# xu-ji/IIC

Hardware: AMD Instinct MI355X
Metric: paired-images/sec, STL10 96x96 ClusterNet5g+IID_loss (higher is better)
Workload: dtype bf16; 1 GPU; STL10 96x96 ClusterNet5g IID+ (cluster_sobel.py train step), batch 660 pairs/GPU, 5 sub-heads, k=70, bf16 MFMA convs / fp32 stem+heads+loss, fused HIP Adam; global_batch_pairs=660, input=96x96x1 grey -> sobel 2ch, parallelism=dp1, streams=2, launch=hip-graph replay: 6 linear graph segments, the two views on two streams

## Files before the change

iic_amd/csrc/conv_igemm_p64.hip:

```cpp
#include "common.h"
#include "conv_plan.h"
#include "conv_tile.h"
#include "../../include/iic_hip.h"

#define P64_BM 256
#define P64_BN 64
#define P64_THREADS 512
#define P64_NT 9
#define P64_CLD P64_BN
#define P64_SC_BYTES(BM_) ((BM_) * P64_CLD * 2)
#define P64_NTAB 4
#define P64_TAB_BYTES(BM_) (P64_NTAB * (BM_) * (4 + 2))

struct P64Walk {
  int n, y, x;
};
__device__ __forceinline__ void p64_walk_init(P64Walk& w, const iic_conv_geom& g, int m) {
  const int plane = g.MY * g.MX;
  w.n = m / plane;
  const int r = m - w.n * plane;
  w.y = r / g.MX;
  w.x = r - w.y * g.MX;
}
__device__ __forceinline__ void p64_walk_advance(P64Walk& w, const iic_conv_geom& g, int d_y, int d_x) {
  w.x += d_x;
  w.y += d_y;
  if (w.x >= g.MX) { w.x -= g.MX; ++w.y; }
  while (w.y >= g.MY) { w.y -= g.MY; ++w.n; }
}
__device__ __forceinline__ void p64_walk_pixels(const P64Walk& w, const iic_conv_geom& g, int& pin,
                                                int& pout) {
  const bool valid = w.n < g.N;
  const int n = valid ? w.n : g.N - 1, y = valid ? w.y : g.MY - 1, x = valid ? w.x : g.MX - 1;
  pin = (n * g.in_Hp + y * g.sy + g.oy) * g.in_Wp + x * g.sx + g.ox;
  pout = valid ? (n * g.out_Hp + y * g.ty + g.py) * g.out_Wp + x * g.tx + g.px : -1;
}

struct P64Row {
  int n, y, x, pin, pout;
};
struct P64Step {
  int d_n, d_y, d_x, MY, MX, pin_step, pin_xw, pin_yw, pout_step, pout_xw, pout_yw;
};
__device__ __forceinline__ void p64_row_init(P64Row& r, const iic_conv_geom& g, int m) {
  P64Walk w;
  p64_walk_init(w, g, m);
  r.n = w.n; r.y = w.y; r.x = w.x;
  r.pin = (w.n * g.in_Hp + w.y * g.sy + g.oy) * g.in_Wp + w.x * g.sx + g.ox;
  r.pout = (w.n * g.out_Hp + w.y * g.ty + g.py) * g.out_Wp + w.x * g.tx + g.px;
}
__device__ __forceinline__ void p64_row_advance(P64Row& r, const P64Step& s) {
  r.n += s.d_n; r.y += s.d_y; r.x += s.d_x; r.pin += s.pin_step; r.pout += s.pout_step;
  const bool cx = r.x >= s.MX;
  r.x -= cx ? s.MX : 0; r.y += cx ? 1 : 0; r.pin += cx ? s.pin_xw : 0; r.pout += cx ? s.pout_xw : 0;
  const bool cy = r.y >= s.MY;
  r.y -= cy ? s.MY : 0; r.n += cy ? 1 : 0; r.pin += cy ? s.pin_yw : 0; r.pout += cy ? s.pout_yw : 0;
}

__device__ __forceinline__ void p64_dma16s(unsigned voff, const unsigned char* sbase, unsigned lds_dst) {
  unsigned keep;
  asm volatile(
      "s_mov_b32 %0, m0\n\ts_mov_b32 m0, %3\n\ts_nop 0\n\tglobal_load_lds_dwordx4 %1, %2\n\ts_mov_b32 m0, %0"
      : "=&s"(keep)
      : "v"(voff), "s"(sbase), "s"(lds_dst)
      : "memory");
}

template <int ABL, int RED, bool FORM>
__global__ __launch_bounds__(512) void conv_igemm_p64_kernel(
    const iic_conv_geom g, const bf16_t* __restrict__ in, const unsigned char* __restrict__ wfrag,
    bf16_t* __restrict__ out, float* __restrict__ stats, const bf16_t* __restrict__ res_grad,
    const bf16_t* __restrict__ res_act, int accumulate, int num_tiles, int pb_bytes, int max_tap_off,
    const bf16_t* __restrict__ red_y, const float* __restrict__ red_coef,
    const bf16_t* __restrict__ red_y2, float* __restrict__ red_stats, float* __restrict__ red_stats2,
    unsigned long long* __restrict__ prof) {
  constexpr bool PROF = (ABL & 8) != 0;
  constexpr bool BK = FORM && RED == 0;
  constexpr int NW = 8, BM = P64_BM;
  constexpr int NWM = BM / 64;
  constexpr int SC_BYTES = BM * P64_CLD * 2, TAB_ROWS = P64_NTAB * BM;
  unsigned long long ph[6] = {0, 0, 0, 0, 0, 0}, t_a = 0, t_b = 0, t_loop = 0;
  extern __shared__ __attribute__((aligned(16))) unsigned char smem_raw[];
  unsigned char* const sP0 = smem_raw;
  unsigned char* const sP1 = smem_raw + pb_bytes;
  bf16_t* const sC = reinterpret_cast<bf16_t*>(smem_raw + 2 * pb_bytes);
  int* const s_pout = reinterpret_cast<int*>(smem_raw + 2 * pb_bytes + SC_BYTES);
  unsigned short* const s_prow = reinterpret_cast<unsigned short*>(s_pout + TAB_ROWS);
  float* const s_red = reinterpret_cast<float*>(sC);

  constexpr int NTH = NW * 64;
  constexpr int NCO = 1;
  const int tid = threadIdx.x, lane = tid & 63;
  const int wave = __builtin_amdgcn_readfirstlane(tid >> 6);
  const int wm = wave >> 1, wn = wave & 1;
  const int l31 = lane & 31, g5 = lane >> 5;
  const uint32_t g5x = (uint32_t)g5 << 4;
  typedef const bf16x8 __attribute__((address_space(3))) * lds_frag_ptr;
  const uint32_t lds_base = __builtin_amdgcn_readfirstlane(
      (uint32_t)(uintptr_t)(__attribute__((address_space(3))) unsigned char*)smem_raw);
  const int M = g.N * g.MY * g.MX;
  const int in_pixels = g.N * g.in_Hp * g.in_Wp;

  const int G = gridDim.x;
  const int wl = xcd_tile_index(blockIdx.x, G);
  const int t0 = (int)(((long)wl * num_tiles) / G), t1 = (int)(((long)(wl + 1) * num_tiles) / G);
  if (t0 >= t1) return;

  const int v_tapoff = g.tap_off[lane & (IIC_MAX_TAPS - 1)];
  const int d_y = BM / g.MX, d_x = BM - d_y * g.MX;

  P64Walk wr, w0, w255;
  p64_walk_init(wr, g, t0 * BM + (tid & (BM - 1)));
  p64_walk_init(w0, g, t0 * BM);
  p64_walk_init(w255, g, t0 * BM + BM - 1);
  int plo_q[3], nblk_q[3];
  auto tabulate = [&](int t) {
    int pin, pout, p0, p255, dummy;
    p64_walk_pixels(w0, g, p0, dummy);
    p64_walk_pixels(w255, g, p255, dummy);
    p0 = __builtin_amdgcn_readfirstlane(p0);
    p255 = __builtin_amdgcn_readfirstlane(p255);
    if (tid < BM) {
      p64_walk_pixels(wr, g, pin, pout);
      s_pout[(t & (P64_NTAB - 1)) * BM + tid] = pout;
      s_prow[(t & (P64_NTAB - 1)) * BM + tid] = (unsigned short)(pin - p0);
    }
    p64_walk_advance(wr, g, d_y, d_x);
    p64_walk_advance(w0, g, d_y, d_x);
    p64_walk_advance(w255, g, d_y, d_x);
    plo_q[0] = plo_q[1];
    nblk_q[0] = nblk_q[1];
    plo_q[1] = plo_q[2];
    nblk_q[1] = nblk_q[2];
    plo_q[2] = p0;
    nblk_q[2] = ((p255 + max_tap_off - p0 + 1) * 128 + 1023) >> 10;
  };
  auto dma_issue = [&](unsigned char* dst, int plo, int nblk) {
    for (int blk = wave; blk < nblk; blk += NW) {
      const int q = blk * 64 + lane;
      const int r = q >> 3;
      const int ls = (q & 7) ^ ((r >> 1) & 7);
      int p = plo + r;
      p = p < in_pixels ? p : in_pixels - 1;
      __builtin_amdgcn_global_load_lds(
          (const __attribute__((address_space(1))) void*)(in + ((long)p * 64 + ls * 8)),
          (__attribute__((address_space(3))) void*)(dst + blk * 1024), 16, 0, 0);
    }
  };

  P64Step stp;
  P64Row rr, r0, r255;
  int pin_last = 0;
  uint32_t lane_src = 0;
  if (BK) {
    const int plane = g.MY * g.MX;
    stp.d_n = BM / plane;
    const int rem = BM - stp.d_n * plane;
    stp.d_y = rem / g.MX;
    stp.d_x = rem - stp.d_y * g.MX;
    stp.MY = g.MY; stp.MX = g.MX;
    stp.pin_step = (stp.d_n * g.in_Hp + stp.d_y * g.sy) * g.in_Wp + stp.d_x * g.sx;
    stp.pin_xw = g.sy * g.in_Wp - g.MX * g.sx;
    stp.pin_yw = (g.in_Hp - g.MY * g.sy) * g.in_Wp;
    stp.pout_step = (stp.d_n * g.out_Hp + stp.d_y * g.ty) * g.out_Wp + stp.d_x * g.tx;
    stp.pout_xw = g.ty * g.out_Wp - g.MX * g.tx;
    stp.pout_yw = (g.out_Hp - g.MY * g.ty) * g.out_Wp;
    pin_last = ((g.N - 1) * g.in_Hp + (g.MY - 1) * g.sy + g.oy) * g.in_Wp + (g.MX - 1) * g.sx + g.ox;
    p64_row_init(rr, g, t0 * BM + (tid & (BM - 1)));
    p64_row_init(r0, g, t0 * BM);
    p64_row_init(r255, g, t0 * BM + BM - 1);
    lane_src = (uint32_t)(lane >> 3) * 128u + (uint32_t)(((lane & 7) ^ (lane >> 4) ^ ((wave & 1) << 2)) << 4);
  }
  auto tabulate1 = [&](int t) {
    const int p0 = r0.n < g.N ? r0.pin : pin_last;
    const int p255 = r255.n < g.N ? r255.pin : pin_last;
    if (wave < BM / 64) {
      const bool valid = rr.n < g.N;
      s_pout[(t & (P64_NTAB - 1)) * BM + tid] = valid ? rr.pout : -1;
      s_prow[(t & (P64_NTAB - 1)) * BM + tid] = (unsigned short)((valid ? rr.pin : pin_last) - p0);
      p64_row_advance(rr, stp);
    }
    p64_row_advance(r0, stp);
    p64_row_advance(r255, stp);
    plo_q[0] = plo_q[1];
    nblk_q[0] = nblk_q[1];
    plo_q[1] = plo_q[2];
    nblk_q[1] = nblk_q[2];
    plo_q[2] = p0;
    nblk_q[2] = ((p255 + max_tap_off - p0 + 1) * 128 + 1023) >> 10;
  };
  auto dma_issue1 = [&](uint32_t dst, int plo, int nblk) {
    const unsigned char* const ing = reinterpret_cast<const unsigned char*>(in);
    for (int blk = wave; blk < nblk; blk += NW) {
      const int rb = plo + blk * 8;
      const unsigned char* src = ing + (long)rb * 128;
      uint32_t vo = lane_src;
      if (rb + 7 >= in_pixels) {
        const int rc = rb < in_pixels ? rb : in_pixels - 1;
        int p = rb + (lane >> 3);
        p = p < in_pixels ? p : in_pixels - 1;
        src = ing + (long)rc * 128;
        vo = (uint32_t)(p - rc) * 128u + (lane_src & 127u);
      }
      p64_dma16s(vo, src, dst + (uint32_t)blk * 1024u);
    }
  };
  int R0[2];

  if (BK) {
    tabulate1(t0);
    tabulate1(t0 + 1);
    __syncthreads();
#pragma unroll
    for (int ms = 0; ms < 2; ++ms) R0[ms] = s_prow[(t0 & (P64_NTAB - 1)) * BM + wm * 64 + ms * 32 + l31];
    dma_issue1(lds_base, plo_q[1], nblk_q[1]);
  } else {
    tabulate(t0);
    tabulate(t0 + 1);
    dma_issue(sP0, plo_q[1], nblk_q[1]);
  }
  u32x4 Bw[P64_NT][NCO][4];
#pragma unroll
  for (int tap = 0; tap < P64_NT; ++tap)
#pragma unroll
    for (int c = 0; c < NCO; ++c) {
      const unsigned char* p = wfrag + ((long)g.tap_w[tap] * 2 + wn + c) * 4096 + lane * 16;
#pragma unroll
      for (int ks = 0; ks < 4; ++ks) Bw[tap][c][ks] = *reinterpret_cast<const u32x4*>(p + ks * 1024);
    }
  f32x2 st_s[NCO], st_ss[NCO];
#pragma unroll
  for (int c = 0; c < NCO; ++c) {
    st_s[c] = f32x2{0.f, 0.f};
    st_ss[c] = f32x2{0.f, 0.f};
  }
  TileRed tr;
  if (RED) tile_red_zero(tr);

  if (PROF) t_loop = __builtin_readcyclecounter();
  for (int t = t0; t < t1; ++t) {
    const int par = (t - t0) & 1;
    unsigned char* const sP = par ? sP1 : sP0;
    if (PROF) t_a = __builtin_readcyclecounter();
    asm volatile("s_waitcnt vmcnt(0)" ::: "memory");
    __syncthreads();
    if (PROF) { t_b = __builtin_readcyclecounter(); ph[0] += t_b - t_a; t_a = t_b; }
    const bool spread = RED == 0 && !res_grad && !res_act && !accumulate;
    if (t > t0 && !(ABL & 2) && !spread)
      igemm_store_tile<P64_BN, BM, NTH, 0, RED, (RED ? 1 : 4)>(sC, s_pout + ((t - 1) & (P64_NTAB - 1)) * BM,
                                                            out, res_grad, res_act, accumulate, P64_BN, 0, tid,
                                                            red_y, red_coef, red_y2, &tr);
    if (PROF) { t_b = __builtin_readcyclecounter(); ph[1] += t_b - t_a; t_a = t_b; }
    if (!BK) {
      if (t + 1 < t1 && !(ABL & 1)) dma_issue(par ? sP0 : sP1, plo_q[2], nblk_q[2]);
      tabulate(t + 2);
    }
    if (PROF) { t_b = __builtin_readcyclecounter(); ph[2] += t_b - t_a; t_a = t_b; }
    if (!BK) {
#pragma unroll
      for (int ms = 0; ms < 2; ++ms)
        R0[ms] = s_prow[(t & (P64_NTAB - 1)) * BM + wm * 64 + ms * 32 + l31];
    }
    const uint32_t pbase = lds_base + (par ? (uint32_t)pb_bytes : 0u);
    const int prow = (int)(pbase >> 7);
    const uint32_t kfix = (pbase >> 4) & 0x40u;
    f32x16 acc[2][NCO];
    constexpr int NTAPS = (ABL & 4) ? 1 : P64_NT;
    auto load_a = [&](int tap, bf16x8 (&a)[2][4]) {
      const int toff = __builtin_amdgcn_readlane(v_tapoff, tap);
      if (FORM) {
        const int toffp = toff + prow;
#pragma unroll
        for (int ms = 0; ms < 2; ++ms) {
          uint32_t tt = (uint32_t)(R0[ms] + toffp) << 3;
          asm volatile("" : "+v"(tt));
          uint32_t u = (tt << 4) | (tt & 0x70u);
          asm volatile("" : "+v"(u));
#pragma unroll
          for (int ks = 0; ks < 4; ++ks)
            a[ms][ks] = *reinterpret_cast<const lds_frag_ptr>((uintptr_t)(u ^ g5x ^ ((uint32_t)(ks << 5) ^ kfix)));
        }
        return;
      }
#pragma unroll
      for (int ms = 0; ms < 2; ++ms) {
        const int R = R0[ms] + toff;
        const int key = (R >> 1) & 7;
        const int base = R * 128 + (((g5 ^ key) & 1) << 4);
        const int kk = (key >> 1) << 5;
#pragma unroll
        for (int ks = 0; ks < 4; ++ks)
          a[ms][ks] = *reinterpret_cast<const bf16x8*>(sP + base + ((ks << 5) ^ kk));
      }
    };
#pragma unroll
    for (int tap = 0; tap < NTAPS; ++tap) {
      bf16x8 a[2][4];
      load_a(tap, a);
      if (BK) {
        if (tap == 0 && t + 1 < t1 && !(ABL & 1)) dma_issue1(lds_base + (par ? 0u : (uint32_t)pb_bytes), plo_q[2], nblk_q[2]);
        if (tap == (NTAPS > 6 ? 6 : NTAPS - 1)) tabulate1(t + 2);
      }
      if (spread && t > t0 && !(ABL & 2)) {
        constexpr int SIT = BM * 8 / NTH;
        constexpr int PER = (SIT + P64_NT - 2) / (P64_NT - 1);
#pragma unroll
        for (int q = 0; q < PER; ++q) {
          const int it = (tap - 1) * PER + q;
          if (tap >= 1 && it < SIT) {
            const int idx = tid + it * NTH;
            const int row = idx >> 3, ch = idx & 7;
            const int po = s_pout[((t - 1) & (P64_NTAB - 1)) * BM + row];
            if (po >= 0)
              *reinterpret_cast<uint4*>(out + (long)po * P64_BN + ch * 8) =
                  *reinterpret_cast<const uint4*>(sC + row * P64_CLD + ch * 8);
          }
        }
      }
#pragma unroll
      for (int ks = 0; ks < 4; ++ks)
#pragma unroll
        for (int c = 0; c < NCO; ++c) {
          const bf16x8 b = __builtin_bit_cast(bf16x8, Bw[tap][c][ks]);
          if (tap == 0 && ks == 0) {
            const f32x16 z = {0.f, 0.f, 0.f, 0.f, 0.f, 0.f, 0.f, 0.f, 0.f, 0.f, 0.f, 0.f, 0.f, 0.f, 0.f, 0.f};
            acc[0][c] = __builtin_amdgcn_mfma_f32_32x32x16_bf16(a[0][ks], b, z, 0, 0, 0);
            acc[1][c] = __builtin_amdgcn_mfma_f32_32x32x16_bf16(a[1][ks], b, z, 0, 0, 0);
          } else {
            acc[0][c] = __builtin_amdgcn_mfma_f32_32x32x16_bf16(a[0][ks], b, acc[0][c], 0, 0, 0);
            acc[1][c] = __builtin_amdgcn_mfma_f32_32x32x16_bf16(a[1][ks], b, acc[1][c], 0, 0, 0);
          }
        }
    }
    if (stats) {
      if ((t + 1) * BM > M) {
#pragma unroll
        for (int ms = 0; ms < 2; ++ms)
#pragma unroll
          for (int r = 0; r < 16; ++r)
            if (t * BM + wm * 64 + ms * 32 + mfma32_row(r, lane) >= M) {
#pragma unroll
              for (int c = 0; c < NCO; ++c) acc[ms][c][r] = 0.f;
            }
      }
#pragma unroll
      for (int c = 0; c < NCO; ++c)
#pragma unroll
        for (int ms = 0; ms < 2; ++ms)
#pragma unroll
          for (int r = 0; r < 16; r += 2) {
            const f32x2 v = {acc[ms][c][r], acc[ms][c][r + 1]};
            st_s[c] += v;
            st_ss[c] += v * v;
          }
    }
    if (PROF) { t_b = __builtin_readcyclecounter(); ph[3] += t_b - t_a; t_a = t_b; }
    asm volatile("s_waitcnt lgkmcnt(0)" ::: "memory");
    __builtin_amdgcn_s_barrier();
    if (PROF) { t_b = __builtin_readcyclecounter(); ph[4] += t_b - t_a; t_a = t_b; }
#pragma unroll
    for (int c = 0; c < NCO; ++c)
#pragma unroll
      for (int ms = 0; ms < 2; ++ms)
#pragma unroll
        for (int r = 0; r < 16; ++r)
          sC[(wm * 64 + ms * 32 + mfma32_row(r, lane)) * P64_CLD + (wn + c) * 32 + l31] = f32_to_bf16(acc[ms][c][r]);
    if (BK && t + 1 < t1) {
#pragma unroll
      for (int ms = 0; ms < 2; ++ms) R0[ms] = s_prow[((t + 1) & (P64_NTAB - 1)) * BM + wm * 64 + ms * 32 + l31];
    }
    if (PROF) { t_b = __builtin_readcyclecounter(); ph[5] += t_b - t_a; }
  }
  if (PROF && prof && tid == 0) {
    unsigned long long* q = prof + (long)blockIdx.x * 8;
#pragma unroll
    for (int i = 0; i < 6; ++i) q[i] = ph[i];
    q[6] = (unsigned long long)(t1 - t0);
    q[7] = __builtin_readcyclecounter() - t_loop;
  }

  __syncthreads();
  if (!(ABL & 2))
    igemm_store_tile<P64_BN, BM, NTH, 0, RED, (RED ? 1 : 4)>(sC, s_pout + ((t1 - 1) & (P64_NTAB - 1)) * BM, out,
                                                          res_grad, res_act, accumulate, P64_BN, 0, tid,
                                                          red_y, red_coef, red_y2, &tr);
  if (RED)
    igemm_red_finish<P64_BN, NTH, RED>(tr, reinterpret_cast<float*>(sC), red_stats, red_stats2, P64_BN,
                                               0, tid);
  if (stats) {
    __syncthreads();
#pragma unroll
    for (int c = 0; c < NCO; ++c) {
      float s1 = st_s[c][0] + st_s[c][1], s2 = st_ss[c][0] + st_ss[c][1];
      s1 += __shfl_xor(s1, 32, 64);
      s2 += __shfl_xor(s2, 32, 64);
      if (lane < 32) {
        s_red[(wm * 2 + 0) * P64_BN + (wn + c) * 32 + lane] = s1;
        s_red[(wm * 2 + 1) * P64_BN + (wn + c) * 32 + lane] = s2;
      }
    }
    __syncthreads();
    if (tid < P64_BN) {
      float a0 = 0.f, a1 = 0.f;
#pragma unroll
      for (int q = 0; q < NWM; ++q) {
        a0 += s_red[(q * 2 + 0) * P64_BN + tid];
        a1 += s_red[(q * 2 + 1) * P64_BN + tid];
      }
      const int stripe = blockIdx.x % IIC_STAT_STRIPES;
      iic_stat_add(stats, stripe, P64_BN, tid, 0, a0);
      iic_stat_add(stats, stripe, P64_BN, tid, 1, a1);
    }
  }
}

#ifdef IIC_DEBUG_HOOKS
static unsigned long long* g_p64_prof = nullptr;
IIC_HOOK void iic_debug_p64_prof(void* buf) { g_p64_prof = (unsigned long long*)buf; }
#else
static constexpr unsigned long long* g_p64_prof = nullptr;
#endif
IIC_SWITCH(g_p64_grid, 0, iic_debug_p64_grid)
IIC_SWITCH(g_p64_form, 1, iic_debug_p64_form)

static long p64_pb_bytes(const iic_conv_geom* g, int bm = P64_BM) {
  return (((long)(bm == 128 ? g->NP : g->NP256) * 128) + 1023) & ~1023L;
}

bool iic_p64_plan(const iic_conv_geom* g, conv_plan* p) {
  if (g->Cin != 64 || g->Cout != 64 || g->ntaps != P64_NT || g->NP256 <= 0 || g->NP256 > 65535) return false;
  if (!igemm_dense_host(g)) return false;
  const long lds = 2 * p64_pb_bytes(g) + P64_SC_BYTES(P64_BM) + P64_TAB_BYTES(P64_BM);
  if (lds > IIC_LDS_BYTES) return false;
  const long nt = ((long)g->N * g->MY * g->MX + P64_BM - 1) / P64_BM;
  const int ncu = g_p64_grid > 0 ? g_p64_grid : iic_num_cus();
  p->kernel = CONV_P64;
  p->mtiles = (int)nt;
  p->grid = nt < ncu ? (int)nt : ncu;
  p->lds_a = (int)p64_pb_bytes(g);
  p->lds = lds;
  return true;
}

int iic_p64_launch(const iic_conv_geom* g, const conv_plan& p, const void* in, const void* wfrag, void* out, float* stats,
                   const void* res_grad, const void* res_act, int accumulate, const void* red_y,
                   const float* red_coef, const void* red_y2, float* red_stats, float* red_stats2,
                   void* stream) {
  const int red = red_y ? (red_y2 ? 2 : 1) : 0;
  const long M = (long)g->N * g->MY * g->MX;
  if (M <= 0) return IIC_ERR_ARG;
  if (M >= (1L << 31) - P64_BM || (long)g->N * g->in_Hp * g->in_Wp >= (1L << 31)) return IIC_ERR_UNSUPPORTED;
  int mto = 0;
  for (int i = 0; i < g->ntaps; ++i) mto = g->tap_off[i] > mto ? g->tap_off[i] : mto;
  int rc = IIC_OK;
#define P64_LAUNCH3(AB_, RD_, FM_)                                                                     \
  rc = iic_launch_lds<conv_igemm_p64_kernel<AB_, RD_, FM_>>(                                           \
      dim3(p.grid), dim3(512), p.lds, (hipStream_t)stream, *g, (const bf16_t*)in,                      \
      (const unsigned char*)wfrag, (bf16_t*)out, stats, (const bf16_t*)res_grad,                       \
      (const bf16_t*)res_act, accumulate, p.mtiles, p.lds_a, mto, (const bf16_t*)red_y, red_coef,      \
      (const bf16_t*)red_y2, red_stats, red_stats2, g_p64_prof)
#ifdef IIC_DEBUG_HOOKS
#define P64_LAUNCH2(AB_, RD_)                                                                          \
  do {                                                                                                 \
    if (g_p64_form) P64_LAUNCH3(AB_, RD_, true);                                                       \
    else P64_LAUNCH3(AB_, RD_, false);                                                                 \
  } while (0)
#else
#define P64_LAUNCH2(AB_, RD_) P64_LAUNCH3(AB_, RD_, true)
#endif
#define P64_LAUNCH(AB_) P64_LAUNCH2(AB_, 0)
  if (red == 1) P64_LAUNCH2(0, 1);
  else if (red == 2) P64_LAUNCH2(0, 2);
  else {
    switch (iic_debug_get_ablate()) {
#ifdef IIC_BD_ABLATIONS
      case 1: P64_LAUNCH(1); break;
      case 2: P64_LAUNCH(2); break;
      case 3: P64_LAUNCH(3); break;
      case 4: P64_LAUNCH(4); break;
      case 7: P64_LAUNCH(7); break;
      case 8: P64_LAUNCH(8); break;
#endif
      default: P64_LAUNCH(0); break;
    }
  }
  return rc ? rc : iic_launch_status();
}
```

iic_amd/csrc/conv_tile.h:

```cpp
#pragma once
#include "common.h"
#include "../../include/iic_hip.h"

__device__ __forceinline__ void igemm_row_pixels(const iic_conv_geom& g, int m, int& pin, int& pout) {
  const int plane = g.MY * g.MX;
  const int mp = g.MP > 0 ? g.MP : plane;
  int n = m / mp;
  int r = m - n * mp;
  const bool valid = n < g.N && r < plane;
  if (n >= g.N) { n = g.N - 1; r = plane - 1; }
  r = r < plane ? r : plane - 1;
  const int y = r / g.MX, x = r - y * g.MX;
  pin = (n * g.in_Hp + y * g.sy + g.oy) * g.in_Wp + x * g.sx + g.ox;
  pout = valid ? (n * g.out_Hp + y * g.ty + g.py) * g.out_Wp + x * g.tx + g.px : -1;
}
__device__ __forceinline__ int igemm_rows(const iic_conv_geom& g) {
  return g.N * (g.MP > 0 ? g.MP : g.MY * g.MX);
}
__device__ __forceinline__ bool igemm_tile_has_invalid(const iic_conv_geom& g, int m0, int bm) {
  const int plane = g.MY * g.MX;
  if (m0 + bm > igemm_rows(g)) return true;
  return g.MP > 0 && g.MP != plane && (m0 % g.MP) + bm > plane;
}
static inline long igemm_rows_host(const iic_conv_geom* g) {
  return (long)g->N * (g->MP > 0 ? g->MP : g->MY * g->MX);
}
static inline bool igemm_dense_host(const iic_conv_geom* g) { return g->MP <= 0 || g->MP == g->MY * g->MX; }

#define ROWB 144
#define PT144_ROWS 7
#define PT144_PIECE (PT144_ROWS * ROWB)
static inline long pt144_bytes(long npix) {
  return ((npix + PT144_ROWS - 1) / PT144_ROWS) * PT144_PIECE + 16;
}

__device__ __forceinline__ int xcd_tile_index(int b, int nwg) {
  const int q = nwg >> 3, r = nwg & 7, xcd = b & 7, idx = b >> 3;
  return (xcd < r ? xcd * (q + 1) : r * (q + 1) + (xcd - r) * q) + idx;
}

template <bool GATHER, int NTHREADS, int NB = 4>
__device__ __forceinline__ void igemm_load_patch(unsigned char* sA, const bf16_t* __restrict__ in,
                                                 int Cin, int c0, int p_lo, int npix,
                                                 int in_pixels, const int* s_pin, int tid) {
  const int n8 = npix * 8;
  for (int base = 0; base < n8; base += NTHREADS * NB) {
    u32x4 v[NB];
#pragma unroll
    for (int u = 0; u < NB; ++u) {
      const int idx = base + u * NTHREADS + tid;
      v[u] = (u32x4){0u, 0u, 0u, 0u};
      if (idx < n8) {
        const long p = GATHER ? (long)s_pin[idx >> 3] : (long)p_lo + (idx >> 3);
        if (p < in_pixels) v[u] = *reinterpret_cast<const u32x4*>(in + (p * Cin + c0 + (idx & 7) * 8));
      }
    }
#pragma unroll
    for (int u = 0; u < NB; ++u) {
      const int idx = base + u * NTHREADS + tid;
      if (idx < n8) *reinterpret_cast<u32x4*>(sA + (idx >> 3) * ROWB + (idx & 7) * 16) = v[u];
    }
  }
}

struct TileRed {
  float s[8], sy[8], sy2[8];
};
__device__ __forceinline__ void tile_red_zero(TileRed& r) {
#pragma unroll
  for (int i = 0; i < 8; ++i) r.s[i] = r.sy[i] = r.sy2[i] = 0.f;
}

template <int BN, int BM, int NTHREADS, int PAD = 8, int RED = 0, int UB = 4>
__device__ __forceinline__ void igemm_store_tile(const bf16_t* sC, const int* s_pout,
                                                 bf16_t* __restrict__ out,
                                                 const bf16_t* __restrict__ res_grad,
                                                 const bf16_t* __restrict__ res_act, int accumulate,
                                                 int Cout, int n0, int tid,
                                                 const bf16_t* __restrict__ red_y = nullptr,
                                                 const float* __restrict__ red_coef = nullptr,
                                                 const bf16_t* __restrict__ red_y2 = nullptr,
                                                 TileRed* red = nullptr) {
  constexpr int CLD = BN + PAD;
  constexpr int CH = BN / 8;
  constexpr int ITERS = (BM * CH + NTHREADS - 1) / NTHREADS;
  constexpr int U = ITERS < UB ? ITERS : UB;
  static_assert(NTHREADS % CH == 0, "a thread must keep its channel chunk");
  const bool add_prev = accumulate & IIC_ACC_ADD, premask = accumulate & IIC_ACC_PREMASK;
  const bool any_in = add_prev || res_grad || res_act;
  const int ch = tid % CH;
  float msc[RED ? 8 : 1], msh[RED ? 8 : 1];
  if (RED && red_coef) {
#pragma unroll
    for (int i = 0; i < 8; ++i) {
      msc[RED ? i : 0] = red_coef[n0 + ch * 8 + i];
      msh[RED ? i : 0] = red_coef[Cout + n0 + ch * 8 + i];
    }
  }
  for (int b0 = 0; b0 < ITERS; b0 += U) {
    long o[U];
    uint4 pv[U], gv[U], av[U], yv[U], zv[U];
#pragma unroll
    for (int u = 0; u < U; ++u) {
      const int idx = tid + (b0 + u) * NTHREADS;
      const int row = idx / CH;
      const int po = (idx < BM * CH) ? s_pout[row] : -1;
      o[u] = po < 0 ? -1 : (long)po * Cout + n0 + ch * 8;
      if (o[u] >= 0) {
        if (add_prev) pv[u] = *reinterpret_cast<const uint4*>(out + o[u]);
        if (res_grad) gv[u] = *reinterpret_cast<const uint4*>(res_grad + o[u]);
        if (res_act) av[u] = *reinterpret_cast<const uint4*>(res_act + o[u]);
        if (RED) yv[u] = *reinterpret_cast<const uint4*>(red_y + o[u]);
        if (RED == 2) zv[u] = *reinterpret_cast<const uint4*>(red_y2 + o[u]);
      }
    }
#pragma unroll
    for (int u = 0; u < U; ++u) {
      if (o[u] < 0) continue;
      const int row = (tid + (b0 + u) * NTHREADS) / CH;
      uint4 v = *reinterpret_cast<const uint4*>(sC + row * CLD + ch * 8);
      if (any_in) {
        uint32_t vv[4] = {v.x, v.y, v.z, v.w};
        float f[8];
#pragma unroll
        for (int i = 0; i < 4; ++i) { f[2 * i] = bf16lo(vv[i]); f[2 * i + 1] = bf16hi(vv[i]); }
        if (add_prev) {
          const uint32_t oo[4] = {pv[u].x, pv[u].y, pv[u].z, pv[u].w};
#pragma unroll
          for (int i = 0; i < 4; ++i) { f[2 * i] += bf16lo(oo[i]); f[2 * i + 1] += bf16hi(oo[i]); }
        }
        if (premask) {
          if (res_grad) {
            const uint32_t gg[4] = {gv[u].x, gv[u].y, gv[u].z, gv[u].w};
#pragma unroll
            for (int i = 0; i < 4; ++i) { f[2 * i] += bf16lo(gg[i]); f[2 * i + 1] += bf16hi(gg[i]); }
          }
          if (res_act) {
            const uint32_t aa[4] = {av[u].x, av[u].y, av[u].z, av[u].w};
#pragma unroll
            for (int i = 0; i < 4; ++i) {
              if (!(bf16lo(aa[i]) > 0.f)) f[2 * i] = 0.f;
              if (!(bf16hi(aa[i]) > 0.f)) f[2 * i + 1] = 0.f;
            }
          }
        } else if (res_grad) {
          const uint32_t gg[4] = {gv[u].x, gv[u].y, gv[u].z, gv[u].w};
          const uint32_t aa[4] = {av[u].x, av[u].y, av[u].z, av[u].w};
#pragma unroll
          for (int i = 0; i < 4; ++i) {
            if (bf16lo(aa[i]) > 0.f) f[2 * i] += bf16lo(gg[i]);
            if (bf16hi(aa[i]) > 0.f) f[2 * i + 1] += bf16hi(gg[i]);
          }
        }
        v = make_uint4(pack_bf16x2(f[0], f[1]), pack_bf16x2(f[2], f[3]), pack_bf16x2(f[4], f[5]),
                       pack_bf16x2(f[6], f[7]));
      }
      *reinterpret_cast<uint4*>(out + o[u]) = v;
      if (RED) {
        const uint32_t gq4[4] = {v.x, v.y, v.z, v.w};
        const uint32_t yy[4] = {yv[u].x, yv[u].y, yv[u].z, yv[u].w};
        float gq[8], yq[8];
#pragma unroll
        for (int i = 0; i < 4; ++i) {
          gq[2 * i] = bf16lo(gq4[i]); gq[2 * i + 1] = bf16hi(gq4[i]);
          yq[2 * i] = bf16lo(yy[i]); yq[2 * i + 1] = bf16hi(yy[i]);
        }
        if (red_coef) {
#pragma unroll
          for (int i = 0; i < 8; ++i)
            if (!(yq[i] * msc[RED ? i : 0] + msh[RED ? i : 0] > 0.f)) gq[i] = 0.f;
        }
#pragma unroll
        for (int i = 0; i < 8; ++i) { red->s[i] += gq[i]; red->sy[i] += gq[i] * yq[i]; }
        if (RED == 2) {
          const uint32_t zz[4] = {zv[u].x, zv[u].y, zv[u].z, zv[u].w};
#pragma unroll
          for (int i = 0; i < 4; ++i) {
            red->sy2[2 * i] += gq[2 * i] * bf16lo(zz[i]);
            red->sy2[2 * i + 1] += gq[2 * i + 1] * bf16hi(zz[i]);
          }
        }
      }
    }
  }
}

template <int BN, int NTHREADS, int RED>
__device__ __forceinline__ void igemm_red_finish(TileRed& r, float* scratch, float* red_stats,
                                                 float* red_stats2, int Cout, int n0, int tid) {
  constexpr int CH = BN / 8, NW = NTHREADS / 64;
  static_assert(64 % CH == 0, "channel chunks must divide the wave");
  const int lane = tid & 63, wave = tid >> 6, ch = tid % CH;
#pragma unroll
  for (int i = 0; i < 8; ++i) {
#pragma unroll
    for (int o = CH; o < 64; o <<= 1) {
      r.s[i] += __shfl_xor(r.s[i], o, 64);
      r.sy[i] += __shfl_xor(r.sy[i], o, 64);
      if (RED == 2) r.sy2[i] += __shfl_xor(r.sy2[i], o, 64);
    }
  }
  __syncthreads();
  if (lane < CH) {
#pragma unroll
    for (int i = 0; i < 8; ++i) {
      scratch[(wave * 3 + 0) * BN + ch * 8 + i] = r.s[i];
      scratch[(wave * 3 + 1) * BN + ch * 8 + i] = r.sy[i];
      if (RED == 2) scratch[(wave * 3 + 2) * BN + ch * 8 + i] = r.sy2[i];
    }
  }
  __syncthreads();
  if (tid < BN) {
    float a0 = 0.f, a1 = 0.f, a2 = 0.f;
    for (int w = 0; w < NW; ++w) {
      a0 += scratch[(w * 3 + 0) * BN + tid];
      a1 += scratch[(w * 3 + 1) * BN + tid];
      if (RED == 2) a2 += scratch[(w * 3 + 2) * BN + tid];
    }
    const int stripe = blockIdx.x % IIC_STAT_STRIPES;
    iic_stat_add(red_stats, stripe, Cout, n0 + tid, 0, a0);
    iic_stat_add(red_stats, stripe, Cout, n0 + tid, 1, a1);
    if (RED == 2) {
      iic_stat_add(red_stats2, stripe, Cout, n0 + tid, 0, a0);
      iic_stat_add(red_stats2, stripe, Cout, n0 + tid, 1, a2);
    }
  }
}
```

Before: 19480 paired-images/sec.

## Prefetch epilogue residual/reduction operands during the MFMA phase of the p64 conv

Adds an AHEAD template variant of the p64 implicit-GEMM conv kernel. It issues global loads for the next tile's epilogue inputs (residual grad, activation, accumulate source, reduction y/y2, coefficients) right after the MFMA loop, before the barrier, then consumes them from registers in a new store routine. For RED kernels the accumulators are packed to bf16 early to free registers. The aim is to hide epilogue global-load latency behind the barrier and LDS writes, at the cost of higher VGPR pressure. It is enabled by default for non-spread, RED 0/1 launches.

```diff
diff --git a/iic_amd/csrc/conv_igemm_p64.hip b/iic_amd/csrc/conv_igemm_p64.hip
--- a/iic_amd/csrc/conv_igemm_p64.hip
+++ b/iic_amd/csrc/conv_igemm_p64.hip
@@ -66,7 +66,7 @@
       : "memory");
 }
 
-template <int ABL, int RED, bool FORM>
+template <int ABL, int RED, bool FORM, bool AHEAD>
 __global__ __launch_bounds__(512) void conv_igemm_p64_kernel(
     const iic_conv_geom g, const bf16_t* __restrict__ in, const unsigned char* __restrict__ wfrag,
     bf16_t* __restrict__ out, float* __restrict__ stats, const bf16_t* __restrict__ res_grad,
@@ -236,6 +236,11 @@
   }
   TileRed tr;
   if (RED) tile_red_zero(tr);
+  const bool spread = RED == 0 && !res_grad && !res_act && !accumulate;
+  constexpr int EPI_ITERS = BM * (P64_BN / 8) / NTH;
+  constexpr int EPI_NS = RED == 0 ? EPI_ITERS : (RED == 1 ? 2 : 1);
+  TileEpi<RED, EPI_NS> epi;
+  const bool epi_ahead = AHEAD && !spread && !(ABL & 2);
 
   if (PROF) t_loop = __builtin_readcyclecounter();
   for (int t = t0; t < t1; ++t) {
@@ -245,11 +250,16 @@
     asm volatile("s_waitcnt vmcnt(0)" ::: "memory");
     __syncthreads();
     if (PROF) { t_b = __builtin_readcyclecounter(); ph[0] += t_b - t_a; t_a = t_b; }
-    const bool spread = RED == 0 && !res_grad && !res_act && !accumulate;
-    if (t > t0 && !(ABL & 2) && !spread)
-      igemm_store_tile<P64_BN, BM, NTH, 0, RED, (RED ? 1 : 4)>(sC, s_pout + ((t - 1) & (P64_NTAB - 1)) * BM,
-                                                            out, res_grad, res_act, accumulate, P64_BN, 0, tid,
-                                                            red_y, red_coef, red_y2, &tr);
+    if (t > t0 && !(ABL & 2) && !spread) {
+      if (AHEAD)
+        igemm_store_consume<P64_BN, BM, NTH, 0>(epi, sC, s_pout + ((t - 1) & (P64_NTAB - 1)) * BM, out, res_grad,
+                                                res_act, accumulate, P64_BN, 0, tid, red_y, red_coef != nullptr, red_y2,
+                                                &tr);
+      else
+        igemm_store_tile<P64_BN, BM, NTH, 0, RED, (RED ? 1 : 4)>(sC, s_pout + ((t - 1) & (P64_NTAB - 1)) * BM,
+                                                              out, res_grad, res_act, accumulate, P64_BN, 0, tid,
+                                                              red_y, red_coef, red_y2, &tr);
+    }
     if (PROF) { t_b = __builtin_readcyclecounter(); ph[1] += t_b - t_a; t_a = t_b; }
     if (!BK) {
       if (t + 1 < t1 && !(ABL & 1)) dma_issue(par ? sP0 : sP1, plo_q[2], nblk_q[2]);
@@ -354,6 +364,23 @@
             st_ss[c] += v * v;
           }
     }
+    constexpr bool PACK = AHEAD && RED != 0;
+    uint32_t accp[2][NCO][8];
+    if (PACK) {
+#pragma unroll
+      for (int c = 0; c < NCO; ++c)
+#pragma unroll
+        for (int ms = 0; ms < 2; ++ms)
+#pragma unroll
+          for (int r = 0; r < 16; r += 2) {
+            uint32_t pk = (uint32_t)f32_to_bf16(acc[ms][c][r]) | ((uint32_t)f32_to_bf16(acc[ms][c][r + 1]) << 16);
+            asm volatile("" : "+v"(pk));
+            accp[ms][c][r >> 1] = pk;
+          }
+    }
+    if (AHEAD)
+      igemm_store_issue<P64_BN, BM, NTH>(epi, epi_ahead, s_pout + (t & (P64_NTAB - 1)) * BM, out, res_grad, res_act,
+                                         accumulate, P64_BN, 0, tid, red_y, red_coef, red_y2);
     if (PROF) { t_b = __builtin_readcyclecounter(); ph[3] += t_b - t_a; t_a = t_b; }
     asm volatile("s_waitcnt lgkmcnt(0)" ::: "memory");
     __builtin_amdgcn_s_barrier();
@@ -364,7 +391,8 @@
       for (int ms = 0; ms < 2; ++ms)
 #pragma unroll
         for (int r = 0; r < 16; ++r)
-          sC[(wm * 64 + ms * 32 + mfma32_row(r, lane)) * P64_CLD + (wn + c) * 32 + l31] = f32_to_bf16(acc[ms][c][r]);
+          sC[(wm * 64 + ms * 32 + mfma32_row(r, lane)) * P64_CLD + (wn + c) * 32 + l31] =
+              PACK ? (bf16_t)(accp[ms][c][r >> 1] >> ((r & 1) * 16)) : f32_to_bf16(acc[ms][c][r]);
     if (BK && t + 1 < t1) {
 #pragma unroll
       for (int ms = 0; ms < 2; ++ms) R0[ms] = s_prow[((t + 1) & (P64_NTAB - 1)) * BM + wm * 64 + ms * 32 + l31];
@@ -380,7 +408,10 @@
   }
 
   __syncthreads();
-  if (!(ABL & 2))
+  if (epi_ahead)
+    igemm_store_consume<P64_BN, BM, NTH, 0>(epi, sC, s_pout + ((t1 - 1) & (P64_NTAB - 1)) * BM, out, res_grad, res_act,
+                                            accumulate, P64_BN, 0, tid, red_y, red_coef != nullptr, red_y2, &tr);
+  else if (!(ABL & 2))
     igemm_store_tile<P64_BN, BM, NTH, 0, RED, (RED ? 1 : 4)>(sC, s_pout + ((t1 - 1) & (P64_NTAB - 1)) * BM, out,
                                                           res_grad, res_act, accumulate, P64_BN, 0, tid,
                                                           red_y, red_coef, red_y2, &tr);
@@ -422,6 +453,7 @@
 #endif
 IIC_SWITCH(g_p64_grid, 0, iic_debug_p64_grid)
 IIC_SWITCH(g_p64_form, 1, iic_debug_p64_form)
+IIC_SWITCH(g_p64_epi_ahead, 1, iic_debug_p64_epi_ahead)
 
 static long p64_pb_bytes(const iic_conv_geom* g, int bm = P64_BM) {
   return (((long)(bm == 128 ? g->NP : g->NP256) * 128) + 1023) & ~1023L;
@@ -453,22 +485,37 @@
   int mto = 0;
   for (int i = 0; i < g->ntaps; ++i) mto = g->tap_off[i] > mto ? g->tap_off[i] : mto;
   int rc = IIC_OK;
-#define P64_LAUNCH3(AB_, RD_, FM_)                                                                     \
-  rc = iic_launch_lds<conv_igemm_p64_kernel<AB_, RD_, FM_>>(                                           \
+#define P64_LAUNCH3(AB_, RD_, FM_, AH_)                                                                \
+  rc = iic_launch_lds<conv_igemm_p64_kernel<AB_, RD_, FM_, AH_>>(                                      \
       dim3(p.grid), dim3(512), p.lds, (hipStream_t)stream, *g, (const bf16_t*)in,                      \
       (const unsigned char*)wfrag, (bf16_t*)out, stats, (const bf16_t*)res_grad,                       \
       (const bf16_t*)res_act, accumulate, p.mtiles, p.lds_a, mto, (const bf16_t*)red_y, red_coef,      \
       (const bf16_t*)red_y2, red_stats, red_stats2, g_p64_prof)
+  const bool ahead = g_p64_epi_ahead && red != 2 && (red || res_grad || res_act || accumulate);
 #ifdef IIC_DEBUG_HOOKS
 #define P64_LAUNCH2(AB_, RD_)                                                                          \
   do {                                                                                                 \
-    if (g_p64_form) P64_LAUNCH3(AB_, RD_, true);                                                       \
-    else P64_LAUNCH3(AB_, RD_, false);                                                                 \
+    if (!g_p64_form) P64_LAUNCH3(AB_, RD_, false, false);                                              \
+    else if (ahead) P64_LAUNCH3(AB_, RD_, true, (RD_ != 2));                                           \
+    else P64_LAUNCH3(AB_, RD_, true, false);                                                           \
   } while (0)
 #else
-#define P64_LAUNCH2(AB_, RD_) P64_LAUNCH3(AB_, RD_, true)
+#define P64_LAUNCH2(AB_, RD_) P64_LAUNCH2_##RD_(AB_)
+#define P64_LAUNCH2_0(AB_)                                                                             \
+  do {                                                                                                 \
+    if (ahead) P64_LAUNCH3(AB_, 0, true, true);                                                        \
+    else P64_LAUNCH3(AB_, 0, true, false);                                                             \
+  } while (0)
+#define P64_LAUNCH2_1(AB_) P64_LAUNCH3(AB_, 1, true, true)
+#define P64_LAUNCH2_2(AB_) P64_LAUNCH3(AB_, 2, true, false)
 #endif
 #define P64_LAUNCH(AB_) P64_LAUNCH2(AB_, 0)
+#ifdef IIC_BD_ABLATIONS
+  if (red && iic_debug_get_ablate() == 8) {
+    if (red == 1) P64_LAUNCH2(8, 1);
+    else P64_LAUNCH2(8, 2);
+  } else
+#endif
   if (red == 1) P64_LAUNCH2(0, 1);
   else if (red == 2) P64_LAUNCH2(0, 2);
   else {
diff --git a/iic_amd/csrc/conv_tile.h b/iic_amd/csrc/conv_tile.h
--- a/iic_amd/csrc/conv_tile.h
+++ b/iic_amd/csrc/conv_tile.h
@@ -69,6 +69,70 @@
 __device__ __forceinline__ void tile_red_zero(TileRed& r) {
 #pragma unroll
   for (int i = 0; i < 8; ++i) r.s[i] = r.sy[i] = r.sy2[i] = 0.f;
+}
+
+__device__ __forceinline__ uint4 igemm_epi_combine(uint4 v, const uint4& pv, const uint4& gv, const uint4& av,
+                                                   bool add_prev, bool premask, bool has_g, bool has_a) {
+  uint32_t vv[4] = {v.x, v.y, v.z, v.w};
+  float f[8];
+#pragma unroll
+  for (int i = 0; i < 4; ++i) { f[2 * i] = bf16lo(vv[i]); f[2 * i + 1] = bf16hi(vv[i]); }
+  if (add_prev) {
+    const uint32_t oo[4] = {pv.x, pv.y, pv.z, pv.w};
+#pragma unroll
+    for (int i = 0; i < 4; ++i) { f[2 * i] += bf16lo(oo[i]); f[2 * i + 1] += bf16hi(oo[i]); }
+  }
+  if (premask) {
+    if (has_g) {
+      const uint32_t gg[4] = {gv.x, gv.y, gv.z, gv.w};
+#pragma unroll
+      for (int i = 0; i < 4; ++i) { f[2 * i] += bf16lo(gg[i]); f[2 * i + 1] += bf16hi(gg[i]); }
+    }
+    if (has_a) {
+      const uint32_t aa[4] = {av.x, av.y, av.z, av.w};
+#pragma unroll
+      for (int i = 0; i < 4; ++i) {
+        if (!(bf16lo(aa[i]) > 0.f)) f[2 * i] = 0.f;
+        if (!(bf16hi(aa[i]) > 0.f)) f[2 * i + 1] = 0.f;
+      }
+    }
+  } else if (has_g) {
+    const uint32_t gg[4] = {gv.x, gv.y, gv.z, gv.w};
+    const uint32_t aa[4] = {av.x, av.y, av.z, av.w};
+#pragma unroll
+    for (int i = 0; i < 4; ++i) {
+      if (bf16lo(aa[i]) > 0.f) f[2 * i] += bf16lo(gg[i]);
+      if (bf16hi(aa[i]) > 0.f) f[2 * i + 1] += bf16hi(gg[i]);
+    }
+  }
+  return make_uint4(pack_bf16x2(f[0], f[1]), pack_bf16x2(f[2], f[3]), pack_bf16x2(f[4], f[5]), pack_bf16x2(f[6], f[7]));
+}
+template <int RED>
+__device__ __forceinline__ void igemm_epi_reduce(const uint4& v, const uint4& yv, const uint4& zv, bool has_coef,
+                                                 const float* msc, const float* msh, TileRed* red) {
+  const uint32_t gq4[4] = {v.x, v.y, v.z, v.w};
+  const uint32_t yy[4] = {yv.x, yv.y, yv.z, yv.w};
+  float gq[8], yq[8];
+#pragma unroll
+  for (int i = 0; i < 4; ++i) {
+    gq[2 * i] = bf16lo(gq4[i]); gq[2 * i + 1] = bf16hi(gq4[i]);
+    yq[2 * i] = bf16lo(yy[i]); yq[2 * i + 1] = bf16hi(yy[i]);
+  }
+  if (has_coef) {
+#pragma unroll
+    for (int i = 0; i < 8; ++i)
+      if (!(yq[i] * msc[RED ? i : 0] + msh[RED ? i : 0] > 0.f)) gq[i] = 0.f;
+  }
+#pragma unroll
+  for (int i = 0; i < 8; ++i) { red->s[i] += gq[i]; red->sy[i] += gq[i] * yq[i]; }
+  if (RED == 2) {
+    const uint32_t zz[4] = {zv.x, zv.y, zv.z, zv.w};
+#pragma unroll
+    for (int i = 0; i < 4; ++i) {
+      red->sy2[2 * i] += gq[2 * i] * bf16lo(zz[i]);
+      red->sy2[2 * i + 1] += gq[2 * i + 1] * bf16hi(zz[i]);
+    }
+  }
 }
 
 template <int BN, int BM, int NTHREADS, int PAD = 8, int RED = 0, int UB = 4>
@@ -185,6 +249,104 @@
   }
 }
 
+template <int RED, int NS>
+struct TileEpi {
+  uint4 xv[NS], av[NS], yv[RED ? NS : 1], zv[RED == 2 ? NS : 1];
+  float msc[RED ? 8 : 1], msh[RED ? 8 : 1];
+};
+__device__ __forceinline__ void igemm_epi_undef(uint4& v) {
+  asm volatile("" : "=v"(v.x), "=v"(v.y), "=v"(v.z), "=v"(v.w));
+}
+template <int BN, int BM, int NTHREADS, int RED, int NS>
+__device__ __forceinline__ void igemm_epi_load_row(TileEpi<RED, NS>& e, int u, const int* s_pout,
+                                                   const bf16_t* __restrict__ out,
+                                                   const bf16_t* __restrict__ res_grad,
+                                                   const bf16_t* __restrict__ res_act, int accumulate, int Cout,
+                                                   int n0, int tid, const bf16_t* __restrict__ red_y,
+                                                   const bf16_t* __restrict__ red_y2) {
+  constexpr int CH = BN / 8;
+  const bf16_t* const xsrc = res_grad ? res_grad : ((accumulate & IIC_ACC_ADD) ? out : nullptr);
+  const int k = u % NS, idx = tid + u * NTHREADS;
+  const int po = (idx < BM * CH) ? s_pout[idx / CH] : -1;
+  if (po >= 0) {
+    const long o = (long)po * Cout + n0 + (tid % CH) * 8;
+    if (xsrc) e.xv[k] = *reinterpret_cast<const uint4*>(xsrc + o);
+    if (res_act) e.av[k] = *reinterpret_cast<const uint4*>(res_act + o);
+    if (RED) e.yv[RED ? k : 0] = *reinterpret_cast<const uint4*>(red_y + o);
+    if (RED == 2) e.zv[RED == 2 ? k : 0] = *reinterpret_cast<const uint4*>(red_y2 + o);
+  }
+}
+template <int BN, int BM, int NTHREADS, int RED, int NS>
+__device__ __forceinline__ void igemm_store_issue(TileEpi<RED, NS>& e, bool on, const int* s_pout,
+                                                  const bf16_t* __restrict__ out,
+                                                  const bf16_t* __restrict__ res_grad,
+                                                  const bf16_t* __restrict__ res_act, int accumulate, int Cout,
+                                                  int n0, int tid, const bf16_t* __restrict__ red_y,
+                                                  const float* __restrict__ red_coef,
+                                                  const bf16_t* __restrict__ red_y2) {
+  constexpr int CH = BN / 8;
+  static_assert(NTHREADS % CH == 0, "a thread must keep its channel chunk");
+#pragma unroll
+  for (int k = 0; k < NS; ++k) {
+    igemm_epi_undef(e.xv[k]);
+    igemm_epi_undef(e.av[k]);
+    if (RED) igemm_epi_undef(e.yv[RED ? k : 0]);
+    if (RED == 2) igemm_epi_undef(e.zv[RED == 2 ? k : 0]);
+  }
+  if (RED) {
+#pragma unroll
+    for (int i = 0; i < 8; ++i) asm volatile("" : "=v"(e.msc[RED ? i : 0]), "=v"(e.msh[RED ? i : 0]));
+  }
+  if (!on) return;
+#pragma unroll
+  for (int u = 0; u < NS; ++u)
+    igemm_epi_load_row<BN, BM, NTHREADS>(e, u, s_pout, out, res_grad, res_act, accumulate, Cout, n0, tid, red_y, red_y2);
+  if (RED && red_coef) {
+    const int ch = tid % CH;
+#pragma unroll
+    for (int i = 0; i < 8; ++i) {
+      e.msc[RED ? i : 0] = red_coef[n0 + ch * 8 + i];
+      e.msh[RED ? i : 0] = red_coef[Cout + n0 + ch * 8 + i];
+    }
+  }
+}
+template <int BN, int BM, int NTHREADS, int PAD, int RED, int NS>
+__device__ __forceinline__ void igemm_store_consume(TileEpi<RED, NS>& e, const bf16_t* sC, const int* s_pout,
+                                                    bf16_t* __restrict__ out,
+                                                    const bf16_t* __restrict__ res_grad,
+                                                    const bf16_t* __restrict__ res_act, int accumulate, int Cout,
+                                                    int n0, int tid, const bf16_t* __restrict__ red_y,
+                                                    bool has_coef, const bf16_t* __restrict__ red_y2, TileRed* red) {
+  constexpr int CLD = BN + PAD;
+  constexpr int CH = BN / 8;
+  constexpr int ITERS = (BM * CH + NTHREADS - 1) / NTHREADS;
+  static_assert(NS >= 1 && NS <= ITERS, "rows in flight");
+  const bool add_prev = accumulate & IIC_ACC_ADD, premask = accumulate & IIC_ACC_PREMASK;
+  const bool has_g = res_grad != nullptr, has_a = res_act != nullptr;
+  const bool any_in = add_prev || has_g || has_a;
+  const int ch = tid % CH;
+#pragma unroll
+  for (int u = 0; u < ITERS; ++u) {
+    const int k = u % NS, idx = tid + u * NTHREADS;
+    const int row = idx / CH;
+    const int po = (idx < BM * CH) ? s_pout[row] : -1;
+    if (po >= 0) {
+      const long o = (long)po * Cout + n0 + ch * 8;
+      uint4 v = *reinterpret_cast<const uint4*>(sC + row * CLD + ch * 8);
+      if (any_in) {
+        uint4 pv = e.xv[k];
+        if (add_prev && has_g) pv = *reinterpret_cast<const uint4*>(out + o);
+        v = igemm_epi_combine(v, pv, e.xv[k], e.av[k], add_prev, premask, has_g, has_a);
+      }
+      *reinterpret_cast<uint4*>(out + o) = v;
+      if (RED) igemm_epi_reduce<RED>(v, e.yv[RED ? k : 0], e.zv[RED == 2 ? k : 0], has_coef, e.msc, e.msh, red);
+    }
+    if (u + NS < ITERS)
+      igemm_epi_load_row<BN, BM, NTHREADS>(e, u + NS, s_pout, out, res_grad, res_act, accumulate, Cout, n0, tid, red_y,
+                                           red_y2);
+  }
+}
+
 template <int BN, int NTHREADS, int RED>
 __device__ __forceinline__ void igemm_red_finish(TileRed& r, float* scratch, float* red_stats,
                                                  float* red_stats2, int Cout, int n0, int tid) {
```

Measured after the change: 19490 paired-images/sec (median of 2 runs). About the same (+0.1%).
